# Ritesh622/Unbiased-Quantization-Distributed-Mean-Estimation

Measured on AMD Instinct MI355X. Metric: quantize+dequantize M-vectors/sec at d=2^20 (1/2/4/8 GPU) + NMSE vs reference, higher is better.
Workload: dtype f32

## Files before the change

unbiased-quantization-distributed-mean-estimation_amd/csrc/uq_unbiased_kernels.h:

```cpp

#ifndef UQ_UNBIASED_KERNELS_H
#define UQ_UNBIASED_KERNELS_H

#include "uq_common.h"

namespace {

constexpr int kQItems = 16;
constexpr int kQTile = kQBlock * kQItems;
constexpr int64_t kStreamMinClients = 256;
constexpr int64_t kSegMinTiles = 1024;

struct AbsOp {
    static constexpr bool kHist = false;
    float den, fm;
    uint32_t *h, *zn;
    __device__ static AbsOp make(const float*, float, int64_t) { return AbsOp{0.f, 0.f, nullptr, nullptr}; }
    __device__ float operator()(float v) const { return fabsf(v); }
    __device__ void apply4(const float (&v)[4], float (&a)[4]) const {
#pragma unroll
        for (int c = 0; c < 4; ++c) a[c] += fabsf(v[c]);
    }
};

// ... 1022 lines not shown
                        S = S + (lowbit(S) ? ev.t1 : ev.t0);
                    } else {
                        for (int k = 0; k < kQItems; ++k) S = S + (double)ev.fr[k];
                    }
                }
                sl.misc[0] = S + lr->last_run;
            }
            __syncthreads();
            P = sl.misc[0];
            __syncthreads();
        } else {
            TileRegs r;
            load_tile<VEC4>(r, x, d, tiles, (uint32_t)idx, tid);
            stage_tile<VEC4>(r, s_x, tid);
            __syncthreads();
            const int64_t t0 = (int64_t)tile * kQTile;
            const int len = (int)((d - t0) < kQTile ? (d - t0) : kQTile);
            const Binade B = binade_of(P);
            TileState st;
            TileVals tv;
            if (len == kQTile)
                tile_pass1<true, true>(s_x, tv, sl, tid, len, dp, fm, B, st);
            else
                tile_pass1<false, true>(s_x, tv, sl, tid, len, dp, fm, B, st);
            double pnext;
            (void)resolve_exact(P, B, st, tv, s_x, sl, tid, pnext);
            __syncthreads();
            P = pnext;
        }
        Pb = (uint64_t)__double_as_longlong(P);
        ++tile;
    }
}

template <bool VEC4, bool WQ, bool WC, bool CVEC>
__global__ void __launch_bounds__(kQBlock)
tile_out_kernel(const float* __restrict__ x, float* __restrict__ out, int8_t* __restrict__ codes,
                int32_t* __restrict__ overflow, int64_t d, int32_t tiles, float fm, const float* __restrict__ Xs,
                float Xval, const float* __restrict__ l1, const uint64_t* __restrict__ pre, int64_t ldo, int64_t ldc) {
    __shared__ __attribute__((aligned(16))) float s_x[kQTile];
    __shared__ float s_tab[kTab];
    __shared__ ScanLds sl;
    const int tid = threadIdx.x;
    const int32_t tile = blockIdx.x;
    const int64_t vec = blockIdx.y;
    TileRegs r;
    load_tile<VEC4>(r, x, d, tiles, (uint32_t)(vec * tiles + tile), tid);
    const float L = l1[vec];
    build_table(s_tab, tid, L, fm);
    stage_tile<VEC4>(r, s_x, tid);
    __syncthreads();
    const int64_t t0 = (int64_t)tile * kQTile;
    const int len = (int)((d - t0) < kQTile ? (d - t0) : kQTile);
    const DivPlan dp = div_plan(L);
    const double P = __longlong_as_double((long long)pre[vec * tiles + tile]);
    const Binade B = binade_of(P);
    TileState st;
    TileVals tv;
    if (len == kQTile)
        tile_pass1<true, true>(s_x, tv, sl, tid, len, dp, fm, B, st);
    else
        tile_pass1<false, true>(s_x, tv, sl, tid, len, dp, fm, B, st);
    double pnext;
    const double base = resolve_exact(P, B, st, tv, s_x, sl, tid, pnext);
    uint32_t cw[4];
    float kmax = 0.0f;
    tile_pass2<WQ, WC>(s_x, tv, s_tab, tid, base, L, fm, Xs ? Xs[vec] : Xval, cw, kmax);
    if (WC) {
        store_codes<CVEC>(codes + vec * ldc + t0, cw, len, tid);
        publish_kmax(kmax, L, overflow, vec, tid);
    }
    __syncthreads();
    if (WQ) store_tile<VEC4>(s_x, out + vec * ldo + t0, len, tid);
}

constexpr int kMeanThreads = 1024;
template <bool VEC4>
__global__ void __launch_bounds__(kMeanThreads)
client_mean_kernel(const float* __restrict__ q, int64_t n, int64_t d, int64_t ld, float n_div, int accumulate,
                   float* __restrict__ est) {
    const int64_t col = ((int64_t)blockIdx.x * blockDim.x + threadIdx.x) * 4;
    if (col >= d) return;
    if (VEC4) {
        float4 e = accumulate ? *reinterpret_cast<const float4*>(est + col) : make_float4(0.f, 0.f, 0.f, 0.f);
        int64_t j = 0;
        for (; j + 8 <= n; j += 8) {
            float4 t[8];
#pragma unroll
            for (int u = 0; u < 8; ++u) t[u] = ld_stream(reinterpret_cast<const float4*>(q + (j + u) * ld + col));
#pragma unroll
            for (int u = 0; u < 8; ++u) {
                e.x += t[u].x / n_div; e.y += t[u].y / n_div;
                e.z += t[u].z / n_div; e.w += t[u].w / n_div;
            }
        }
        for (; j < n; ++j) {
            const float4 t = *reinterpret_cast<const float4*>(q + j * ld + col);
            e.x += t.x / n_div; e.y += t.y / n_div; e.z += t.z / n_div; e.w += t.w / n_div;
        }
        *reinterpret_cast<float4*>(est + col) = e;
    } else {
        const int cnt = (int)((d - col) < 4 ? (d - col) : 4);
        for (int k = 0; k < cnt; ++k) {
            float e = accumulate ? est[col + k] : 0.f;
            for (int64_t j = 0; j < n; ++j) e += q[j * ld + col + k] / n_div;
            est[col + k] = e;
        }
    }
}

constexpr int kDecChunk = 4096;
constexpr int kMeanClients = 32;

__device__ __forceinline__ float decode_one(int8_t c, const float* tab) {
    const int ci = (int)c;
    const int k = ci ^ (ci >> 31);
    return __uint_as_float(__float_as_uint(tab[k]) ^ ((uint32_t)ci & 0x80000000u));
}

template <bool VEC>
__global__ void __launch_bounds__(256)
codes_decode_kernel(const int8_t* __restrict__ codes, const float* __restrict__ l1, int64_t d, float fm,
                    float* __restrict__ out) {
    __shared__ float tab[128];
    const int64_t vec = blockIdx.y;
    const int tid = threadIdx.x;
    const float L = l1[vec];
    if (tid < 128) tab[tid] = (L * (float)tid) / fm;
    __syncthreads();
    const int64_t i0 = (int64_t)blockIdx.x * kDecChunk + (int64_t)tid * 16;
    const int8_t* cr = codes + vec * d;
    float* orow = out + vec * d;
    if (VEC && i0 + 16 <= d) {
        const uint4 w = *reinterpret_cast<const uint4*>(cr + i0);
        const uint32_t ws[4] = {w.x, w.y, w.z, w.w};
#pragma unroll
        for (int k4 = 0; k4 < 4; ++k4) {
            float o[4];
#pragma unroll
            for (int c = 0; c < 4; ++c) o[c] = decode_one((int8_t)((ws[k4] >> (8 * c)) & 0xFF), tab);
            *reinterpret_cast<float4*>(orow + i0 + 4 * k4) = make_float4(o[0], o[1], o[2], o[3]);
        }
    } else {
        for (int64_t i = i0; i < i0 + 16 && i < d; ++i) orow[i] = decode_one(cr[i], tab);
    }
}

constexpr int kMeanCpt = 8;
constexpr int kCodesMeanThreads = 512;
constexpr int kMeanUnroll = 16;
static_assert(kMeanClients == 2 * kMeanUnroll, "two code batches per table group");

__device__ __forceinline__ void mean_load_batch(uint2 (&w)[kMeanUnroll], const int8_t* cp, int64_t ldc) {
#pragma unroll
    for (int u = 0; u < kMeanUnroll; ++u) {
        const u32x2v t = __builtin_nontemporal_load(reinterpret_cast<const u32x2v*>(cp + (int64_t)u * ldc));
        w[u] = make_uint2(t.x, t.y);
    }
}

__device__ __forceinline__ void mean_add_batch(float (&e)[kMeanCpt], const uint2 (&w)[kMeanUnroll],
                                               const float (*tabn)[256], int jj) {
#pragma unroll
    for (int u = 0; u < kMeanUnroll; ++u) {
        const float* tb = tabn[jj + u];
#pragma unroll
        for (int k = 0; k < 4; ++k) e[k] += tb[(w[u].x >> (8 * k)) & 0xFF];
#pragma unroll
        for (int k = 0; k < 4; ++k) e[4 + k] += tb[(w[u].y >> (8 * k)) & 0xFF];
    }
}

__device__ __forceinline__ void mean_build_tables(float (*tabn)[256], const float* __restrict__ l1,
                                                  const int32_t* __restrict__ kmaxv, int64_t j0, int nb, int wid,
                                                  int lane, float fm, float n_div) {
    for (int jj = wid; jj < nb; jj += kCodesMeanThreads / kWave) {
        const float L = l1[j0 + jj];
        const int km = min(127, max(0, kmaxv[j0 + jj]));
        for (int k = lane; k <= km; k += kWave) {
            const float v = ((L * (float)k) / fm) / n_div;
            tabn[jj][k] = v;
            tabn[jj][255 - k] = -v;
        }
    }
}

__device__ __forceinline__ void mean_add_bytes(float (&e)[kMeanCpt], const int8_t* __restrict__ codes, int64_t ldc,
                                               const float (*tabn)[256], int64_t j0, int nb, int64_t i0, int64_t d) {
    for (int jj = 0; jj < nb; ++jj)
        for (int k = 0; k < kMeanCpt; ++k)
            if (i0 + k < d) e[k] += tabn[jj][(uint8_t)codes[(j0 + jj) * ldc + i0 + k]];
}

__device__ __forceinline__ uint32_t mean_ovf_mask(const int32_t* __restrict__ kmaxv, int64_t j0, int nb) {
    uint32_t mk = 0;
    for (int jj = 0; jj < nb; ++jj) mk |= (kmaxv[j0 + jj] > 127 ? 1u : 0u) << jj;
    return mk;
}

__device__ __forceinline__ void mean_add_mixed(float (&e)[kMeanCpt], const int8_t* __restrict__ codes, int64_t ldc,
                                            const float* __restrict__ q, int64_t ldq, const float (*tabn)[256],
                                            uint32_t ovf, int64_t j0, int nb, int64_t i0, int64_t d, float n_div) {
    for (int jj = 0; jj < nb; ++jj) {
        const int64_t j = j0 + jj;
        if ((ovf >> jj) & 1u) {
            for (int k = 0; k < kMeanCpt; ++k)
                if (i0 + k < d) e[k] += q[j * ldq + i0 + k] / n_div;
        } else {
            for (int k = 0; k < kMeanCpt; ++k)
                if (i0 + k < d) e[k] += tabn[jj][(uint8_t)codes[j * ldc + i0 + k]];
        }
    }
}

template <bool VEC, bool ALL = false>
__global__ void __launch_bounds__(kCodesMeanThreads)
codes_mean_kernel(const int8_t* __restrict__ codes, int64_t ldc, const float* __restrict__ l1,
                  const int32_t* __restrict__ kmaxv, int64_t n, int64_t d, float fm, float n_div, int accumulate,
                  float* __restrict__ est, const float* __restrict__ q, int64_t ldq) {
    __shared__ float tabn[kMeanClients][256];
    __shared__ uint32_t s_ovf;
    const int tid = threadIdx.x;
    const int lane = tid & (kWave - 1);
    const int wid = __builtin_amdgcn_readfirstlane(tid / kWave);
    const int64_t i0 = ((int64_t)blockIdx.x * kCodesMeanThreads + tid) * kMeanCpt;
    const bool full = ALL || (VEC && i0 + kMeanCpt <= d);
    float e[kMeanCpt];
#pragma unroll
    for (int k = 0; k < kMeanCpt; ++k) e[k] = (accumulate && i0 + k < d) ? est[i0 + k] : 0.0f;
    bool any = false;
    if (q) {
        if (tid == 0) s_ovf = 0u;
        __syncthreads();
        bool a = false;
        for (int64_t j = tid; j < n; j += kCodesMeanThreads) a = a || kmaxv[j] > 127;
        if (a) s_ovf = 1u;
        __syncthreads();
        any = s_ovf != 0u;
    }
    const int64_t groups = n / kMeanClients;
    if (any) {
        for (int64_t j0 = 0; j0 < n; j0 += kMeanClients) {
            const int nb = (int)min((int64_t)kMeanClients, n - j0);
            const uint32_t ovf = mean_ovf_mask(kmaxv, j0, nb);
            __syncthreads();
            mean_build_tables(tabn, l1, kmaxv, j0, nb, wid, lane, fm, n_div);
            __syncthreads();
            mean_add_mixed(e, codes, ldc, q, ldq, tabn, ovf, j0, nb, i0, d, n_div);
        }
    } else {
    const int8_t* cbase = codes + (full ? i0 : 0);
    uint2 wa[kMeanUnroll], wb[kMeanUnroll];
    if (VEC && groups > 0) mean_load_batch(wa, cbase, ldc);
    for (int64_t g = 0; g < groups; ++g) {
        const int64_t j0 = g * kMeanClients;
        __syncthreads();
        mean_build_tables(tabn, l1, kmaxv, j0, kMeanClients, wid, lane, fm, n_div);
        __syncthreads();
        if (VEC) {
            mean_load_batch(wb, cbase + (j0 + kMeanUnroll) * ldc, ldc);
            if (full) mean_add_batch(e, wa, tabn, 0);
            const int64_t jn = (j0 + kMeanClients + kMeanUnroll <= n) ? j0 + kMeanClients : n - kMeanUnroll;
            mean_load_batch(wa, cbase + jn * ldc, ldc);
            if (full) mean_add_batch(e, wb, tabn, kMeanUnroll);
        }
        if (!full) mean_add_bytes(e, codes, ldc, tabn, j0, kMeanClients, i0, d);
    }
    const int64_t jr = groups * kMeanClients;
    const int nr = (int)(n - jr);
    if (nr > 0) {
        __syncthreads();
        mean_build_tables(tabn, l1, kmaxv, jr, nr, wid, lane, fm, n_div);
        __syncthreads();
        if (full) {
            for (int jj = 0; jj < nr; ++jj) {
                const uint2 w = *reinterpret_cast<const uint2*>(codes + (jr + jj) * ldc + i0);
#pragma unroll
                for (int k = 0; k < 4; ++k) e[k] += tabn[jj][(w.x >> (8 * k)) & 0xFF];
#pragma unroll
                for (int k = 0; k < 4; ++k) e[4 + k] += tabn[jj][(w.y >> (8 * k)) & 0xFF];
            }
        } else {
            mean_add_bytes(e, codes, ldc, tabn, jr, nr, i0, d);
        }
    }
    }
    if (full) {
        *reinterpret_cast<float4*>(est + i0) = make_float4(e[0], e[1], e[2], e[3]);
        *reinterpret_cast<float4*>(est + i0 + 4) = make_float4(e[4], e[5], e[6], e[7]);
    } else {
        for (int k = 0; k < kMeanCpt; ++k)
            if (i0 + k < d) est[i0 + k] = e[k];
    }
}

constexpr int kNibMax = 7;
constexpr int64_t kNibAlign = kCodesMeanThreads * kMeanCpt;

__device__ __forceinline__ void nib_load_batch(uint32_t (&w)[kMeanUnroll], const uint8_t* cp, int64_t ldn) {
#pragma unroll
    for (int u = 0; u < kMeanUnroll; ++u) w[u] = __builtin_nontemporal_load(reinterpret_cast<const uint32_t*>(cp + (int64_t)u * ldn));
}

__device__ __forceinline__ void nib_add_batch(float (&e)[kMeanCpt], const uint32_t (&w)[kMeanUnroll],
                                              const float (*tab)[16], int jj) {
#pragma unroll
    for (int u = 0; u < kMeanUnroll; ++u) {
        const float* tb = tab[jj + u];
#pragma unroll
        for (int k = 0; k < kMeanCpt; ++k) e[k] += tb[(w[u] >> (4 * k)) & 0xFu];
    }
}

constexpr int kNibChunk = 1024;
__device__ __forceinline__ void nib_build_tables(float (*tab)[16], const float* __restrict__ l1,
                                                 const int32_t* __restrict__ kmaxv, int64_t j0, int nb, float fm,
                                                 float n_div) {
    for (int e = threadIdx.x; e < nb * 8; e += kCodesMeanThreads) {
        const int jj = e >> 3, k = e & 7;
        const float L = l1[j0 + jj];
        const int km = min(kNibMax, max(0, kmaxv[j0 + jj]));
        if (k <= km) {
            const float v = ((L * (float)k) / fm) / n_div;
            tab[jj][k] = v;
            tab[jj][15 - k] = -v;
        }
    }
}

__global__ void __launch_bounds__(kCodesMeanThreads)
nibbles_mean_kernel(const uint8_t* __restrict__ nib, int64_t ldn, const float* __restrict__ l1,
                    const int32_t* __restrict__ kmaxv, int64_t n, int64_t d, float fm, float n_div, int accumulate,
                    float* __restrict__ est, const float* __restrict__ q, int64_t ldq) {
    __shared__ float tab[kNibChunk][16];
    __shared__ uint32_t s_ovf;
    const int tid = threadIdx.x;
    const int64_t i0 = ((int64_t)blockIdx.x * kCodesMeanThreads + tid) * kMeanCpt;
    float e[kMeanCpt];
    if (accumulate) {
        const float4 a = *reinterpret_cast<const float4*>(est + i0), b = *reinterpret_cast<const float4*>(est + i0 + 4);
        e[0] = a.x; e[1] = a.y; e[2] = a.z; e[3] = a.w; e[4] = b.x; e[5] = b.y; e[6] = b.z; e[7] = b.w;
    } else {
#pragma unroll
        for (int k = 0; k < kMeanCpt; ++k) e[k] = 0.0f;
    }
    if (tid == 0) s_ovf = 0u;
    __syncthreads();
    bool a = false;
    for (int64_t j = tid; j < n; j += kCodesMeanThreads) a = a || kmaxv[j] > kNibMax;
    if (a) s_ovf = 1u;
    __syncthreads();
    const bool any = s_ovf != 0u;
    const uint8_t* cbase = nib + i0 / 2;
    for (int64_t c0 = 0; c0 < n; c0 += kNibChunk) {
        const int nc = (int)min((int64_t)kNibChunk, n - c0);
        __syncthreads();
        nib_build_tables(tab, l1, kmaxv, c0, nc, fm, n_div);
        __syncthreads();
        const int full = any ? 0 : nc / kMeanClients * kMeanClients;
        if (full > 0) {
            uint32_t wa[kMeanUnroll], wb[kMeanUnroll];
            const uint8_t* cb = cbase + c0 * ldn;
            nib_load_batch(wa, cb, ldn);
            for (int g = 0; g < full; g += kMeanClients) {
                nib_load_batch(wb, cb + (int64_t)(g + kMeanUnroll) * ldn, ldn);
                nib_add_batch(e, wa, tab, g);
                const int gn = (g + kMeanClients + kMeanUnroll <= nc) ? g + kMeanClients : nc - kMeanUnroll;
                nib_load_batch(wa, cb + (int64_t)gn * ldn, ldn);
                nib_add_batch(e, wb, tab, g + kMeanUnroll);
            }
        }
        for (int jj = full; jj < nc; ++jj) {
            const int64_t j = c0 + jj;
            if (kmaxv[j] > kNibMax) {
                const float4 a4 = *reinterpret_cast<const float4*>(q + j * ldq + i0);
                const float4 b4 = *reinterpret_cast<const float4*>(q + j * ldq + i0 + 4);
                const float qq[kMeanCpt] = {a4.x, a4.y, a4.z, a4.w, b4.x, b4.y, b4.z, b4.w};
#pragma unroll
                for (int k = 0; k < kMeanCpt; ++k) e[k] += qq[k] / n_div;
            } else {
                const uint32_t w = *reinterpret_cast<const uint32_t*>(cbase + j * ldn);
#pragma unroll
                for (int k = 0; k < kMeanCpt; ++k) e[k] += tab[jj][(w >> (4 * k)) & 0xFu];
            }
        }
    }
    *reinterpret_cast<float4*>(est + i0) = make_float4(e[0], e[1], e[2], e[3]);
    *reinterpret_cast<float4*>(est + i0 + 4) = make_float4(e[4], e[5], e[6], e[7]);
}

}

#endif
```

Before: 0.4206.

## Use byte-indexed pair lookup tables with double-buffered LDS in nibble mean kernel

Replaces the per-nibble 16-entry table lookup with a 256-entry pair table per client, so one byte of codes fetches two dequantized values (f32x2) per LDS read, halving LDS lookups. Pair tables are double-buffered in shared memory and built cooperatively while the previous batch is accumulated. Code-word prefetch is interleaved into the accumulate loop, and the global overflow pre-scan is replaced by per-chunk overflow detection during table build. It adds extra __syncthreads per group, a larger LDS footprint (64KB pair tables) that may cut occupancy, and XOR-swizzled slots to reduce bank conflicts.

After: 0.4271 (median of 6 runs). +1.5%, better.

```diff
diff --git a/unbiased-quantization-distributed-mean-estimation_amd/csrc/uq_unbiased_kernels.h b/unbiased-quantization-distributed-mean-estimation_amd/csrc/uq_unbiased_kernels.h
--- a/unbiased-quantization-distributed-mean-estimation_amd/csrc/uq_unbiased_kernels.h
+++ b/unbiased-quantization-distributed-mean-estimation_amd/csrc/uq_unbiased_kernels.h
@@ -1348,28 +1348,106 @@
     for (int u = 0; u < kMeanUnroll; ++u) w[u] = __builtin_nontemporal_load(reinterpret_cast<const uint32_t*>(cp + (int64_t)u * ldn));
 }
 
-__device__ __forceinline__ void nib_add_batch(float (&e)[kMeanCpt], const uint32_t (&w)[kMeanUnroll],
-                                              const float (*tab)[16], int jj) {
+constexpr int kPairClients = kMeanUnroll;
+constexpr int kNibChunk = 1024;
+constexpr int kNibRefill = 4;
+static_assert(kCodesMeanThreads == 32 * kPairClients, "32 lanes build one client's pair entries");
+static_assert(2 * kPairClients * 256 * sizeof(f32x2) == 65536, "pair rows are 16-bit DS immediates");
+
+__device__ __forceinline__ uint32_t pair_slot(uint32_t b) { return b ^ (b >> 5); }
+__device__ __forceinline__ uint32_t pair_slots4(uint32_t w) { return w ^ ((w >> 5) & 0x07070707u); }
+
+struct NibLds {
+    f32x2 pair[2][kPairClients][256];
+    float tab[kNibChunk][16];
+    int32_t km[kNibChunk];
+    uint32_t ovf;
+};
+
+constexpr int kNibRows = kNibChunk / kCodesMeanThreads;
+struct NibRows {
+    float L[kNibRows];
+    int32_t kmx[kNibRows];
+};
+
+__device__ __forceinline__ NibRows nib_fetch_rows(const float* __restrict__ l1, const int32_t* __restrict__ kmaxv,
+                                                  int64_t c0, int nc) {
+    NibRows r;
+#pragma unroll
+    for (int i = 0; i < kNibRows; ++i) {
+        const int64_t j = c0 + min((int)threadIdx.x + i * kCodesMeanThreads, nc - 1);
+        r.L[i] = l1[j];
+        r.kmx[i] = kmaxv[j];
+    }
+    return r;
+}
+
+__device__ __forceinline__ bool nib_build_tables(NibLds& s, const NibRows& r, int nc, float fm, float n_div) {
+    bool ovf = false;
+#pragma unroll
+    for (int i = 0; i < kNibRows; ++i) {
+        const int jj = threadIdx.x + i * kCodesMeanThreads;
+        ovf = ovf || (jj < nc && r.kmx[i] > kNibMax);
+        float v[8];
+#pragma unroll
+        for (int k = 0; k < 8; ++k) v[k] = ((r.L[i] * (float)k) / fm) / n_div;
+        f32x4* row = reinterpret_cast<f32x4*>(s.tab[jj]);
+        row[0] = f32x4{v[0], v[1], v[2], v[3]};
+        row[1] = f32x4{v[4], v[5], v[6], v[7]};
+        row[2] = f32x4{-v[7], -v[6], -v[5], -v[4]};
+        row[3] = f32x4{-v[3], -v[2], -v[1], -v[0]};
+        s.km[jj] = min(kNibMax, max(0, r.kmx[i]));
+    }
+    return ovf;
+}
+
+struct PairSrc {
+    float lo;
+    float mag[8];
+    int km;
+};
+
+__device__ __forceinline__ PairSrc pair_fetch(const NibLds& s, int jg) {
+    const int jj = jg + (threadIdx.x >> 5), c = threadIdx.x & 15;
+    PairSrc p;
+    const int km = s.km[jj];
+    const f32x4 a = *reinterpret_cast<const f32x4*>(&s.tab[jj][0]), b = *reinterpret_cast<const f32x4*>(&s.tab[jj][4]);
+    p.lo = s.tab[jj][c];
+    p.mag[0] = a.x; p.mag[1] = a.y; p.mag[2] = a.z; p.mag[3] = a.w;
+    p.mag[4] = b.x; p.mag[5] = b.y; p.mag[6] = b.z; p.mag[7] = b.w;
+    p.km = (c <= km || c >= 15 - km) ? km : -1;
+    return p;
+}
+
+template <int R>
+__device__ __forceinline__ void pair_store(NibLds& s, const PairSrc& p) {
+    const int row = threadIdx.x >> 5, c = threadIdx.x & 15;
+    const bool top = (threadIdx.x & 16) != 0;
+#pragma unroll
+    for (int l = 0; l <= kNibMax; ++l) {
+        if (l <= p.km) {
+            const uint32_t h = top ? 15 - l : l;
+            s.pair[R][row][pair_slot(h << 4 | c)] = f32x2{p.lo, top ? -p.mag[l] : p.mag[l]};
+        }
+    }
+}
+
+template <int R>
+__device__ __forceinline__ void nib_pair_add(float (&e)[kMeanCpt], uint32_t (&w)[kMeanUnroll], const NibLds& s,
+                                             const uint8_t* next, int64_t ldn) {
 #pragma unroll
     for (int u = 0; u < kMeanUnroll; ++u) {
-        const float* tb = tab[jj + u];
-#pragma unroll
-        for (int k = 0; k < kMeanCpt; ++k) e[k] += tb[(w[u] >> (4 * k)) & 0xFu];
-    }
-}
-
-constexpr int kNibChunk = 1024;
-__device__ __forceinline__ void nib_build_tables(float (*tab)[16], const float* __restrict__ l1,
-                                                 const int32_t* __restrict__ kmaxv, int64_t j0, int nb, float fm,
-                                                 float n_div) {
-    for (int e = threadIdx.x; e < nb * 8; e += kCodesMeanThreads) {
-        const int jj = e >> 3, k = e & 7;
-        const float L = l1[j0 + jj];
-        const int km = min(kNibMax, max(0, kmaxv[j0 + jj]));
-        if (k <= km) {
-            const float v = ((L * (float)k) / fm) / n_div;
-            tab[jj][k] = v;
-            tab[jj][15 - k] = -v;
+        const uint32_t x = pair_slots4(w[u]);
+#pragma unroll
+        for (int k = 0; k < 4; ++k) {
+            const f32x2 v = s.pair[R][u][(x >> (8 * k)) & 0xFFu];
+            e[2 * k] += v.x;
+            e[2 * k + 1] += v.y;
+        }
+        if (u % kNibRefill == kNibRefill - 1) {
+#pragma unroll
+            for (int r = u + 1 - kNibRefill; r <= u; ++r)
+                w[r] = __builtin_nontemporal_load(reinterpret_cast<const uint32_t*>(next + (int64_t)r * ldn));
         }
     }
 }
@@ -1378,10 +1456,14 @@
 nibbles_mean_kernel(const uint8_t* __restrict__ nib, int64_t ldn, const float* __restrict__ l1,
                     const int32_t* __restrict__ kmaxv, int64_t n, int64_t d, float fm, float n_div, int accumulate,
                     float* __restrict__ est, const float* __restrict__ q, int64_t ldq) {
-    __shared__ float tab[kNibChunk][16];
-    __shared__ uint32_t s_ovf;
+    __shared__ NibLds s;
     const int tid = threadIdx.x;
     const int64_t i0 = ((int64_t)blockIdx.x * kCodesMeanThreads + tid) * kMeanCpt;
+    const uint8_t* cbase = nib + i0 / 2;
+    uint32_t wa[kMeanUnroll], wb[kMeanUnroll];
+    auto batch = [&](int64_t c0, int nc, int b) {
+        return cbase + (c0 + max(0, min(b * kMeanUnroll, nc - kMeanUnroll))) * ldn;
+    };
     float e[kMeanCpt];
     if (accumulate) {
         const float4 a = *reinterpret_cast<const float4*>(est + i0), b = *reinterpret_cast<const float4*>(est + i0 + 4);
@@ -1390,33 +1472,39 @@
 #pragma unroll
         for (int k = 0; k < kMeanCpt; ++k) e[k] = 0.0f;
     }
-    if (tid == 0) s_ovf = 0u;
-    __syncthreads();
-    bool a = false;
-    for (int64_t j = tid; j < n; j += kCodesMeanThreads) a = a || kmaxv[j] > kNibMax;
-    if (a) s_ovf = 1u;
-    __syncthreads();
-    const bool any = s_ovf != 0u;
-    const uint8_t* cbase = nib + i0 / 2;
     for (int64_t c0 = 0; c0 < n; c0 += kNibChunk) {
         const int nc = (int)min((int64_t)kNibChunk, n - c0);
+        const NibRows rows = nib_fetch_rows(l1, kmaxv, c0, nc);
+        const int64_t ldc = nc >= kMeanUnroll ? ldn : 0;
+        nib_load_batch(wa, nc >= kMeanUnroll ? batch(c0, nc, 0) : cbase + (c0 + nc - 1) * ldn, ldc);
+        nib_load_batch(wb, nc >= kMeanUnroll ? batch(c0, nc, 1) : cbase + (c0 + nc - 1) * ldn, ldc);
+        const uint32_t chunk_id = (uint32_t)(c0 / kNibChunk) + 1u;
+        if (c0 == 0 && tid == 0) s.ovf = 0u;
         __syncthreads();
-        nib_build_tables(tab, l1, kmaxv, c0, nc, fm, n_div);
+        if (nib_build_tables(s, rows, nc, fm, n_div)) s.ovf = chunk_id;
         __syncthreads();
-        const int full = any ? 0 : nc / kMeanClients * kMeanClients;
-        if (full > 0) {
-            uint32_t wa[kMeanUnroll], wb[kMeanUnroll];
-            const uint8_t* cb = cbase + c0 * ldn;
-            nib_load_batch(wa, cb, ldn);
-            for (int g = 0; g < full; g += kMeanClients) {
-                nib_load_batch(wb, cb + (int64_t)(g + kMeanUnroll) * ldn, ldn);
-                nib_add_batch(e, wa, tab, g);
-                const int gn = (g + kMeanClients + kMeanUnroll <= nc) ? g + kMeanClients : nc - kMeanUnroll;
-                nib_load_batch(wa, cb + (int64_t)gn * ldn, ldn);
-                nib_add_batch(e, wb, tab, g + kMeanUnroll);
+        const int groups = s.ovf == chunk_id ? 0 : nc / kPairClients;
+        if (groups > 0) {
+            PairSrc ps = pair_fetch(s, 0);
+            pair_store<0>(s, ps);
+            if (groups > 1) ps = pair_fetch(s, kPairClients);
+            int g = 0;
+            for (; g + 1 < groups; g += 2) {
+                __syncthreads();
+                pair_store<1>(s, ps);
+                if (g + 2 < groups) ps = pair_fetch(s, (g + 2) * kPairClients);
+                nib_pair_add<0>(e, wa, s, batch(c0, nc, g + 2), ldn);
+                __syncthreads();
+                if (g + 2 < groups) pair_store<0>(s, ps);
+                if (g + 3 < groups) ps = pair_fetch(s, (g + 3) * kPairClients);
+                nib_pair_add<1>(e, wb, s, batch(c0, nc, g + 3), ldn);
             }
-        }
-        for (int jj = full; jj < nc; ++jj) {
+            if (g < groups) {
+                __syncthreads();
+                nib_pair_add<0>(e, wa, s, batch(c0, nc, g + 2), ldn);
+            }
+        }
+        for (int jj = groups * kPairClients; jj < nc; ++jj) {
             const int64_t j = c0 + jj;
             if (kmaxv[j] > kNibMax) {
                 const float4 a4 = *reinterpret_cast<const float4*>(q + j * ldq + i0);
@@ -1427,7 +1515,7 @@
             } else {
                 const uint32_t w = *reinterpret_cast<const uint32_t*>(cbase + j * ldn);
 #pragma unroll
-                for (int k = 0; k < kMeanCpt; ++k) e[k] += tab[jj][(w >> (4 * k)) & 0xFu];
+                for (int k = 0; k < kMeanCpt; ++k) e[k] += s.tab[jj][(w >> (4 * k)) & 0xFu];
             }
         }
     }
```
